# z-prize/2022-entries

Measured on AMD Instinct MI355X. Metric: BLS12-377 G1 MSM point-scalar pairs/s, higher is better.
Workload: dtype u32

## Files before the change

2022-entries_amd/csrc/host_test_api.cpp:

```cpp
#include <stdint.h>
#include <stdio.h>

static long g_check_failures = 0;
static char g_first_failure[256];
static void msm_check_fail(const char* file, int line, const char* cond) {
  if (g_check_failures++ == 0) snprintf(g_first_failure, sizeof g_first_failure, "%s:%d %s", file, line, cond);
}
#define MSM_CHECK(cond) do { if (!(cond)) msm_check_fail(__FILE__, __LINE__, #cond); } while (0)
#define MSM_CHECK_COL_BEGIN() unsigned __int128 chk_col_ = col
#define MSM_CHECK_COL_ADD(x) chk_col_ += (x)
#define MSM_CHECK_COL_END(col) MSM_CHECK(chk_col_ == (unsigned __int128)(col))

#include "host_curve.hpp"
#include "te.hpp"

using namespace msm;

template <class F>
static void t_fe_mul(const uint8_t* a, const uint8_t* b, uint8_t* out) {
  Modulus<F> md;
  Fe x, y, z;
  uint32_t wa[12], wb[12], wo[12];
  memcpy(wa, a, 48);
  memcpy(wb, b, 48);
// ... 655 lines not shown
  uint32_t s[8];
  memcpy(s, scalar, 32);
  const uint32_t levels = fb_levels((uint32_t)w);
  for (uint32_t j = 0; j < levels; j++) out[j] = fb_digit(s, j, (uint32_t)w);
  return (int)levels;
}
int ht_fb_table_level(int curve, const uint8_t* g_img, int w, int level, uint8_t* out, size_t stride) {
  if (!g_img || !out || w < 1 || w > (int)FB_MAX_WINDOW || level < 0 || level >= (int)fb_levels((uint32_t)w) || stride % 4) return -1;
  DISPATCH_C(curve, t_fb_table_level, g_img, w, level, out, stride)
}
int ht_fb_mul(int curve, const uint8_t* g_img, int w, const uint8_t* scalars, size_t n, unsigned flags, uint8_t* out, size_t stride) {
  if (!g_img || (n && (!scalars || !out)) || w < 1 || w > (int)FB_MAX_WINDOW || stride % 4 || (flags & ~3u)) return -1;
  DISPATCH_C(curve, t_fb_mul, g_img, w, scalars, n, flags, out, stride)
}
}
```

2022-entries_amd/csrc/launch.hpp:

```cpp
#pragma once
#include <hip/hip_runtime.h>

#include "host_curve.hpp"
#include "msm_types.hpp"
#include "partition_plan.hpp"
#include "te.hpp"

namespace msm {

template <class E>
struct Launch {
  using El = typename E::T;
  static hipError_t convert_bases(const uint8_t* in, size_t stride, uint32_t n, bool serialized, AffineDevT<El>* out, uint8_t* inf,
                                  hipStream_t st);
  static hipError_t accumulate(const uint2* entries, const uint32_t* n_real, uint32_t K,
                               const AffineDevT<El>* bases, SegOutT<El> out, uint32_t nlanes, hipStream_t st, bool paired = false);
  static hipError_t segreduce(const XyzzDevT<El>* in_slots, const uint32_t* in_keys, uint32_t n_in, uint32_t K, SegOutT<El> out,
                              uint32_t nlanes, uint32_t quad_limit, hipStream_t st, bool paired = false);
  static hipError_t pre_double(const AffineDevT<El>* in, const uint8_t* inf_in, uint32_t n, uint32_t c, XyzzDevT<El>* out, hipStream_t st);
  static hipError_t pre_normalize(const XyzzDevT<El>* in, uint32_t n, uint32_t J, El* prefix, AffineDevT<El>* out, uint8_t* inf_out,
                                  hipStream_t st);
  static hipError_t bucket_reduce(bool first, const XyzzDevT<El>* in_a, const XyzzDevT<El>* in_x, uint32_t n_per_win, uint32_t L,
                                  uint32_t chunks, uint32_t windows, uint32_t out_stride, XyzzDevT<El>* out_a, XyzzDevT<El>* out_x, hipStream_t st,
                                  bool paired = false);
// ... 26 lines not shown
                               const TeAffineDev* bases, SegOut out, uint32_t nlanes, uint32_t* flags, hipStream_t st);
  static hipError_t segreduce(const XyzzDev* in_slots, const uint32_t* in_keys, uint32_t n_in, uint32_t K, SegOut out, uint32_t nlanes,
                              uint32_t quad_limit, uint32_t* flags, hipStream_t st);
  static hipError_t bucket_reduce(bool first, const XyzzDev* in_a, const XyzzDev* in_x, uint32_t n_per_win, uint32_t L, uint32_t chunks,
                                  uint32_t windows, uint32_t out_stride, XyzzDev* out_a, XyzzDev* out_x, uint32_t* flags, hipStream_t st);
  static hipError_t reduce_scan_step(const XyzzDev* in, const XyzzDev* in2, XyzzDev* out, uint32_t nb, uint32_t windows, uint32_t d, uint32_t mode,
                                     uint32_t quad_limit, uint32_t* flags, hipStream_t st);
  static hipError_t sum_bases(const TeAffineDev* bases, const uint8_t* inf, uint32_t first, uint32_t n, uint32_t per_lane, SegOut out, uint32_t nlanes,
                              uint32_t* flags, hipStream_t st);
};

struct PartLaunch {
  static int run(int scalar_field, int scalar_mode, const uint32_t* d_scalars, const uint8_t* d_inf, const PartPlan& p, const PartBuffers& b,
                 hipStream_t st, hipEvent_t mid, hipError_t& err);
  static hipError_t debug_finish(const PartPlan& p, const PartBuffers& b, const uint32_t* slot_keys, uint32_t nslots, hipStream_t st, char* what,
                                 size_t what_len, uint64_t* checks_done);
};

extern template struct Launch<Bls12_377_G1::E>;
extern template struct Launch<Bls12_381_G1::E>;
extern template struct Launch<Bls12_377_G2::E>;
extern template struct Launch<Bls12_381_G2::E>;
extern template struct LaunchPair<Bls12_377_G2::E>;
extern template struct LaunchPair<Bls12_381_G2::E>;

}
```

2022-entries_amd/csrc/msm_engine.hip:

```cpp
#include <hip/hip_runtime.h>

#include <algorithm>
#include <cstdarg>
#include <cstdio>
#include <cstdlib>
#include <cstring>
#include <string.h>
#include <strings.h>

#include <dlfcn.h>

#include <chrono>
#include <condition_variable>
#include <deque>
#include <functional>
#include <memory>
#include <mutex>
#include <stdexcept>
#include <thread>
#include <type_traits>
#include <string>
#include <vector>

#include "../../include/mi355_msm.h"
// ... 225 lines not shown
  return t;
}

struct Plan {
  uint32_t c, windows, half, keybits;
  uint32_t bucket_windows;
  uint32_t levels;
  uint32_t anchor;
  uint64_t entries;
  uint32_t K, nlanes;
  uint32_t segK;
  uint32_t logL0, logL;
  uint32_t T0;
  uint32_t L0;
  uint32_t scan_nb;
  bool reduce_scan;
  bool scan_direct;
};

}

#ifndef MSM_G2_PAIRED_DEFAULT
#define MSM_G2_PAIRED_DEFAULT 31
#endif
constexpr long kDefaultG2Paired = MSM_G2_PAIRED_DEFAULT;

struct RcclState;

struct mi355_msm_ctx {
  int curve = 0;
// ... 23 lines not shown
  long opt_assume_subgroup = 0;
  long opt_anchor = 1;
  bool anchor_armed = false;
  struct AnchorSum {
    size_t n;
    int shift;
    std::vector<uint8_t> pt;
  };
  std::vector<AnchorSum> anchor_sums;
  uint64_t anchor_sums_computed = 0;
  float anchor_sum_ms = 0;
  uint32_t last_anchor = kNoAnchor;
  long opt_reduce_log_chunk = 0, opt_reduce_log_chunk0 = 0;
  long opt_reduce_scan = -1;
  long opt_reduce_fill = 0;
  long opt_twisted_edwards = 1;
  DevBuf te_bases, flags;
  uint32_t* h_flags = nullptr;
  bool te_active = false;
  bool sw_level0_only = false;
  uint64_t te_fallbacks = 0;
  uint32_t te_fallback_streak = 0;
  uint64_t te_demotions = 0;
  uint64_t oom_backoffs = 0;
  uint64_t peer_stagings = 0;
  long opt_force_peer_staging = 0;
  uint32_t last_bucket_windows = 0, last_l1_bits = 0, last_l1_bins = 0, last_passes = 0;
  uint32_t auto_levels = 0;
  uint64_t debug_checks = 0;
  size_t chunk_cap = 0;
  size_t fitted_chunk = 0;
  bool fitted_tables = false;
  uint32_t fitted_c = 0;
  long opt_mem_limit = 0;
  long inject_alloc_failures = 0;
  uint32_t quad_limit = LaunchTe::kDefaultQuadLimit;
  long opt_g2_paired = kDefaultG2Paired;
  std::vector<mi355_msm_ctx*> shards;
  std::vector<size_t> shard_lo;
  long opt_combine = 0;
  RcclState* rccl = nullptr;
  uint64_t rccl_exchanges = 0;
  uint32_t pre_c = 0, pre_windows = 0;
  bool bases_serialized = false;
// ... 60 lines not shown
    if (opt_reduce_log_chunk0) p.logL0 = (uint32_t)opt_reduce_log_chunk0;
    p.logL0 = std::min<uint32_t>(p.logL0, p.c - 1 ? p.c - 1 : 1);
    p.reduce_scan = opt_reduce_scan != 0;
    const uint32_t scan_log = opt_reduce_scan_log ? (uint32_t)opt_reduce_scan_log : 12;
    p.scan_direct = p.reduce_scan && p.half <= (1u << scan_log);
    if (p.reduce_scan && !p.scan_direct) {
      const uint32_t need = ilog2_floor(p.half) - scan_log;
      if (need > 9 || (need > 8 && p.bucket_windows < 8))
        p.reduce_scan = false;
      else if (p.logL0 < need)
        p.logL0 = need;
    }
    p.L0 = 1u << p.logL0;
    p.T0 = ceil_div(p.half, p.L0);
    p.scan_nb = p.T0;
    if (p.reduce_scan && !p.scan_direct && !opt_reduce_log_chunk && !opt_reduce_log_chunk0) {
      const uint64_t kSimds = 1024;
      const uint64_t fill = opt_reduce_fill > 0 ? (uint64_t)opt_reduce_fill : 1;
      const uint64_t waves = ((uint64_t)p.bucket_windows * p.T0 + 63) / 64;
      if (waves < fill * kSimds && p.T0 >= 1024) {
        const uint32_t t_fit = (uint32_t)(fill * kSimds * 64 / p.bucket_windows);
        if (t_fit > p.T0 && t_fit < 2 * fill * p.T0) {
          const uint32_t L = ceil_div(p.half, t_fit);
          if (L >= 8 && L < p.L0) {
            p.L0 = L;
            p.T0 = ceil_div(p.half, L);
            while (p.scan_nb < p.T0) p.scan_nb *= 2;
          }
        }
      }
    }
    return p;
  }
};

namespace {
// ... 248 lines not shown
    const uint64_t sw = (uint64_t)ts.levels * n * 128 * el, inf = (uint64_t)ts.levels * n;
    const uint64_t te_b = te ? (uint64_t)ts.levels * n * sizeof(TeAffineDev) : 0;
    const uint64_t build = te ? 3 * n * 128 + te_b + n * (224 + 56) : sw + n * (224 + 56) * el;
    mi355_msm_ctx tmp;
    tmp.curve = ctx->curve;
    tmp.pre_c = ts.c;
    tmp.pre_windows = ts.levels;
    tmp.opt_window_bits = ctx->opt_window_bits;
    tmp.opt_assume_subgroup = ctx->opt_assume_subgroup;
    tmp.opt_anchor = ctx->opt_anchor;
    tmp.opt_carry = ctx->opt_carry;
    tmp.opt_lane_entries = ctx->opt_lane_entries;
    tmp.opt_seg_entries = ctx->opt_seg_entries;
    tmp.opt_reduce_scan = ctx->opt_reduce_scan;
    tmp.opt_reduce_fill = ctx->opt_reduce_fill;
    const Plan p = tmp.plan(std::min(n, (size_t)1 << 26));
    const uint64_t steady = (te ? n * 128 * el + te_b : sw) + inf + work_bytes(p, el) + n * 32;
    const uint64_t need = std::max(build + inf, steady);
    if (need + (need >> 4) <= avail) return want;
  }
  return -1;
}

bool build_tables_te_streamed(mi355_msm_ctx* ctx, const uint8_t* d_raw, size_t n, size_t stride, int want_levels, hipStream_t st) {
  using C = Bls12_377_G1;
  using E = C::E;
  if (ctx->opt_precompute == 2 && ctx->inject_alloc_failures > 0) {
    ctx->inject_alloc_failures--;
    throw HipFailure((int)hipErrorOutOfMemory, "table allocation failed: out of memory (injected by the inject_alloc_failures test hook)");
  }
// ... 220 lines not shown
  const AffineDev* bases = ctx->bases.as<AffineDev>();
  const uint8_t* inf = ctx->inf.as<uint8_t>();
  uint32_t* flags = ctx->flags.as<uint32_t>();

  HIP_OK(hipEventRecord(ev[0], st));
  PartBuffers gb{};
  gb.entries[0] = ctx->entries[0].as<uint2>();
  gb.entries[1] = ctx->entries[1].as<uint2>();
  gb.matrix = ctx->part_matrix.as<uint32_t>();
  gb.partial = ctx->part_partial.as<uint32_t>();
  gb.segs[0] = ctx->part_segs[0].as<PartSeg>();
  gb.segs[1] = ctx->part_segs[1].as<PartSeg>();
  gb.subjob_first = ctx->part_subjobs.as<uint32_t>();
  gb.counts = ctx->part_counts.as<uint32_t>();
  gb.totals = ctx->part_totals.as<uint32_t>();
  hipError_t gerr = hipSuccess;
  const int scalar_mode = ctx->opt_scalars_montgomery ? SCALARS_FROM_MONT : ctx->opt_scalars_to_montgomery ? SCALARS_TO_MONT : SCALARS_PLAIN;
  const int sorted = PartLaunch::run((ctx->curve == MI355_BLS12_381_G1 || ctx->curve == MI355_BLS12_381_G2) ? 1 : 0, scalar_mode, d_scalars, inf, gp, gb, st,
                                     ev[1], gerr);
  HIP_OK(gerr);
  const uint2* entries = gb.entries[sorted];
  const uint32_t* n_real = gb.totals;
  const bool carry_in = TE && carry && !carry->first;
  if (!carry_in) HIP_OK(hipMemsetAsync(ctx->buckets.p, 0, nbuckets * sizeof(XyzzDev), st));
  HIP_OK(hipEventRecord(ev[2], st));

  SegOut so{ctx->buckets.as<XyzzDev>(), ctx->slots[0].as<XyzzDev>(), ctx->slot_keys[0].as<uint32_t>()};
  so.carry_in = carry_in ? 1u : 0u;
  if constexpr (TE)
    HIP_OK(LaunchTe::accumulate(entries, n_real, p.K, ctx->te_bases.as<TeAffineDev>(), so, p.nlanes, flags, st));
  else
    HIP_OK(Launch<E>::accumulate(entries, n_real, p.K, bases, so, p.nlanes, st, (ctx->opt_g2_paired & 1) != 0));
  HIP_OK(hipEventRecord(ev[3], st));
#ifdef MSM_DEBUG
  {
    char what[320];
    HIP_OK(PartLaunch::debug_finish(gp, gb, ctx->slot_keys[0].as<uint32_t>(), 2 * p.nlanes, st, what, sizeof what, &ctx->debug_checks));
    if (what[0]) throw HipFailure(-2, what);
  }
#endif

  uint32_t n_in = 2 * p.nlanes;
  int cur = 0;
  if (p.nlanes > 1) {
    for (;;) {
      uint32_t nl = ceil_div(n_in, p.segK);
      if (nl > 1 && 2 * (uint64_t)nl >= n_in) bad_arg("fragment merge would not shrink (%u slots, fan-in %u)", n_in, p.segK);
      SegOut o{ctx->buckets.as<XyzzDev>(), ctx->slots[cur ^ 1].as<XyzzDev>(), ctx->slot_keys[cur ^ 1].as<uint32_t>()};
      if constexpr (TE)
        HIP_OK(LaunchTe::segreduce(ctx->slots[cur].as<XyzzDev>(), ctx->slot_keys[cur].as<uint32_t>(), n_in, p.segK, o, nl, ctx->quad_limit, flags, st));
      else
        HIP_OK(Launch<E>::segreduce(ctx->slots[cur].as<XyzzDev>(), ctx->slot_keys[cur].as<uint32_t>(), n_in, p.segK, o, nl, ctx->quad_limit, st,
// ... 37 lines not shown
    HostTail<E>::set_inf(out);
    return true;
  }

  const XyzzDev* sums_src = nullptr;
  uint32_t sums_stride = 1;
  if (p.reduce_scan) {
    uint32_t nb = p.half;
    XyzzDev* bufs[2] = {bucket_src, ctx->red_a[0].as<XyzzDev>()};
    const XyzzDev* a_sums = nullptr;
    if (!p.scan_direct) {
      if (p.scan_nb != p.T0) {
        HIP_OK(hipMemsetAsync(ctx->red_a[0].p, 0, (size_t)p.bucket_windows * p.scan_nb * sizeof(XyzzDev), st));
        HIP_OK(hipMemsetAsync(ctx->red_x[0].p, 0, (size_t)p.bucket_windows * p.scan_nb * sizeof(XyzzDev), st));
      }
      if constexpr (TE)
        HIP_OK(LaunchTe::bucket_reduce(true, nullptr, bucket_src, p.half, p.L0, p.T0, p.bucket_windows, p.scan_nb,
                                       ctx->red_a[0].as<XyzzDev>(), ctx->red_x[0].as<XyzzDev>(), flags, st));
      else
        HIP_OK(Launch<E>::bucket_reduce(true, nullptr, bucket_src, p.half, p.L0, p.T0, p.bucket_windows, p.scan_nb,
                                        ctx->red_a[0].as<XyzzDev>(), ctx->red_x[0].as<XyzzDev>(), st, (ctx->opt_g2_paired & 2) != 0));
      nb = p.scan_nb;
      a_sums = ctx->red_a[0].as<XyzzDev>();
      bufs[0] = ctx->red_x[0].as<XyzzDev>();
      bufs[1] = ctx->red_x[1].as<XyzzDev>();
    }
    int cur = 0;
    auto step = [&](uint32_t d, uint32_t mode) {
      if constexpr (TE)
        HIP_OK(LaunchTe::reduce_scan_step(bufs[cur], a_sums, bufs[cur ^ 1], nb, p.bucket_windows, d, mode, ctx->quad_limit, flags, st));
      else
        HIP_OK(Launch<E>::reduce_scan_step(bufs[cur], a_sums, bufs[cur ^ 1], nb, p.bucket_windows, d, mode, ctx->quad_limit, st, (ctx->opt_g2_paired & 8) != 0));
      cur ^= 1;
    };
    for (uint32_t d = 1; d < nb; d <<= 1) step(d, 0);
    if (a_sums) step(0, 2);
// ... 952 lines not shown
    } else if (k == "reduce_scan_log") {
      if (value != 0 && (value < 6 || value > 18)) bad_arg("reduce_scan_log %ld out of range [6, 18]", value);
      ctx->opt_reduce_scan_log = value;
    } else if (k == "quad_limit") {
      if (value < 0 || value > (1L << 24)) bad_arg("quad_limit %ld out of range [0, 2^24]", value);
      ctx->quad_limit = (uint32_t)value;
    } else if (k == "g2_paired") {
      if (value < 0 || value > 31) bad_arg("g2_paired %ld out of range [0, 31]", value);
      ctx->opt_g2_paired = value;
    } else if (k == "reduce_scan") {
      if (value < -1 || value > 1) bad_arg("reduce_scan %ld out of range [-1, 1]", value);
      ctx->opt_reduce_scan = value;
    } else if (k == "reduce_fill") {
      if (value < 0 || value > 4) bad_arg("reduce_fill %ld out of range [0, 4]", value);
      ctx->opt_reduce_fill = value;
    } else if (k == "reduce_log_chunk0") {
      if (value < 0 || value > 7) bad_arg("reduce_log_chunk0 %ld out of range [1, 7]", value);
      ctx->opt_reduce_log_chunk0 = value;
    } else if (k == "twisted_edwards") {
      ctx->opt_twisted_edwards = value != 0;
    } else if (k == "precompute") {
      if (value < 0 || value > 2) bad_arg("precompute %ld out of range [0, 2]", value);
      ctx->opt_precompute = value;
    } else if (k == "table_levels") {
      if (value < 0 || value > 64) bad_arg("table_levels %ld out of range [0, 64]", value);
      ctx->opt_table_levels = value;
    } else if (k == "scalars_montgomery") {
      if (value != 0 && ctx->opt_scalars_to_montgomery) bad_arg("scalars_montgomery and scalars_to_montgomery exclude each other");
      ctx->opt_scalars_montgomery = value != 0;
    } else if (k == "scalars_to_montgomery") {
// ... 148 lines not shown
      uint32_t v = 0;
      if (ctx->part_totals.p) {
        ensure_device(ctx);
        HIP_OK(hipDeviceSynchronize());
        HIP_OK(hipMemcpy(&v, ctx->part_totals.p, sizeof v, hipMemcpyDeviceToHost));
      }
      *value = v;
    } else if (k == "anchor_sums")
      *value = ctx->anchor_sums_computed;
    else if (k == "anchor_sum_us")
      *value = (uint64_t)(ctx->anchor_sum_ms * 1000.0f);
    else if (k == "oom_backoffs")
      *value = ctx->oom_backoffs;
    else if (k == "debug_checks")
      *value = ctx->debug_checks;
    else if (k == "chunk_cap")
      *value = ctx->chunk_cap;
    else if (k == "device")
      *value = (uint64_t)ctx->device;
    else if (k == "bases")
      *value = ctx->nbases;
    else if (k == "table_levels")
      *value = ctx->pre_c ? ctx->pre_windows : (ctx->nbases ? 1 : 0);
    else if (k == "table_window_bits")
      *value = ctx->pre_c;
    else if (k == "base_bytes")
      *value = ctx->bases.bytes + ctx->te_bases.bytes + ctx->inf.bytes;
    else if (k == "bucket_windows")
      *value = ctx->last_bucket_windows;
    else if (k == "l1_bits")
// ... 196 lines not shown
```

2022-entries_amd/csrc/partition.hip:

```cpp
#include "launch.hpp"
#include "partition.hpp"

namespace msm {

int PartLaunch::run(int scalar_field, int scalar_mode, const uint32_t* d_scalars, const uint8_t* d_inf, const PartPlan& p, const PartBuffers& b,
                    hipStream_t st, hipEvent_t mid, hipError_t& err) {
  if (scalar_field == 1) {
    if (scalar_mode == SCALARS_FROM_MONT) return part_run<Bls12_381_Fr, SCALARS_FROM_MONT>(d_scalars, d_inf, p, b, st, mid, err);
    if (scalar_mode == SCALARS_TO_MONT) return part_run<Bls12_381_Fr, SCALARS_TO_MONT>(d_scalars, d_inf, p, b, st, mid, err);
    return part_run<Bls12_381_Fr, SCALARS_PLAIN>(d_scalars, d_inf, p, b, st, mid, err);
  }
  if (scalar_mode == SCALARS_FROM_MONT) return part_run<Bls12_377_Fr, SCALARS_FROM_MONT>(d_scalars, d_inf, p, b, st, mid, err);
  if (scalar_mode == SCALARS_TO_MONT) return part_run<Bls12_377_Fr, SCALARS_TO_MONT>(d_scalars, d_inf, p, b, st, mid, err);
  return part_run<Bls12_377_Fr, SCALARS_PLAIN>(d_scalars, d_inf, p, b, st, mid, err);
}

hipError_t PartLaunch::debug_finish(const PartPlan& p, const PartBuffers& b, const uint32_t* slot_keys, uint32_t nslots, hipStream_t st, char* what,
                                    size_t what_len, uint64_t* checks_done) {
  if (what && what_len) what[0] = 0;
#ifdef MSM_DEBUG
  uint32_t* const dbg = b.totals + 4;
  const uint32_t key_limit = p.bsets * p.half;
  hipLaunchKernelGGL(k_dbg_check_slots, dim3(part_ceil_div(nslots ? nslots : 1, 256)), dim3(256), 0, st, slot_keys, nslots, key_limit, dbg);
  hipError_t e = hipStreamSynchronize(st);
  if (e != hipSuccess) return e;
  uint32_t h[4 + DBG_WORDS];
  e = hipMemcpy(h, b.totals, sizeof h, hipMemcpyDeviceToHost);
  if (e != hipSuccess) return e;
  const uint32_t* v = h + 4;
  if (checks_done) *checks_done += v[DBG_CHECKS];
  static const char* const names[] = {"", "segment table has a gap or an overlap", "segment table does not end at the entry total",
                                      "an entry carries key bits its level has already resolved", "sorted keys decrease", "a key is out of range",
                                      "a value names a base outside this chunk", "a slot key after the accumulation is neither KEY_NONE nor a valid key"};
  if (v[DBG_DIGITS] != h[0])
    snprintf(what, what_len, "MSM_DEBUG: %u entries were grouped but the scalars hold %u non-zero digits", h[0], v[DBG_DIGITS]);
  else
    for (int i = DBG_SEG_GAP; i <= DBG_SLOT_KEY; i++)
      if (v[i]) {
        snprintf(what, what_len, "MSM_DEBUG: %s (%u violations; n = %u, c = %u, %u windows)", names[i], v[i], p.n, p.c, p.windows);
        break;
      }
#else
  (void)p; (void)b; (void)slot_keys; (void)nslots; (void)st; (void)what_len; (void)checks_done;
#endif
  return hipSuccess;
}

}
```

2022-entries_amd/csrc/partition.hpp:

```cpp
#pragma once
#include <hip/hip_runtime.h>
#include <stdint.h>

#include <algorithm>

#include "digits.hpp"
#include "partition_plan.hpp"

namespace msm {

__device__ __forceinline__ void lds_barrier() {
#ifdef PART_FULL_BARRIER
  __syncthreads();
#else
  asm volatile("s_waitcnt lgkmcnt(0)\n\ts_barrier" ::: "memory");
#endif
}

__device__ __forceinline__ uint32_t wave_incl_scan(uint32_t v) {
#pragma unroll
  for (int d = 1; d < 64; d <<= 1) {
    const uint32_t u = __shfl_up(v, d, 64);
    if ((int)(threadIdx.x & 63) >= d) v += u;
  }
// ... 437 lines not shown
      uint2 e = stage[j];
      const uint32_t hi = e.y >> 16;
      e.y &= 0xffffu;
#ifdef PART_EXP_L1_NOSTORE
      if (e.x == 0x12345678u && e.y == 0x9abcu) out[0] = e;
#elif defined(PART_EXP_L1_OUT4)
      reinterpret_cast<uint32_t*>(out)[offs[hi] + j] = e.x;
#else
      out[offs[hi] + j] = e;
#endif
    }
  }
}


__device__ __forceinline__ bool subjob_range(const PartSeg* __restrict__ segs, const uint32_t* __restrict__ subjob_first, uint32_t nsegs,
                                             uint32_t j, uint32_t& seg, uint32_t& beg, uint32_t& end) {
  if (j >= subjob_first[nsegs]) return false;
  uint32_t lo = 0, hi = nsegs;
  while (hi - lo > 1) {
    const uint32_t mid = (lo + hi) >> 1;
    if (subjob_first[mid] <= j) lo = mid; else hi = mid;
  }
  while (lo + 1 < nsegs && subjob_first[lo + 1] <= j) lo++;
  seg = lo;
  const PartSeg s = segs[seg];
  const uint32_t k = j - subjob_first[seg];
  beg = s.start + k * PART_SUBJOB;
  end = min(s.start + s.len, beg + PART_SUBJOB);
  return beg < end;
// ... 7 lines not shown
  for (uint32_t j = blockIdx.x; j < nsub; j += gridDim.x) {
    uint32_t seg, beg, end;
    const bool live = subjob_range(segs, subjob_first, pp.nsegs, j, seg, beg, end);
    if (!live || part_fused_takes(segs[seg].len)) continue;
    for (uint32_t b = threadIdx.x; b < nb; b += 1024) hist[b] = 0;
    __syncthreads();
    for (uint32_t e = beg + threadIdx.x; e < end; e += 1024) atomicAdd(&hist[(in[e].y >> shift) & (nb - 1)], 1u);
    __syncthreads();
    uint32_t* row = counts + (size_t)j * nb;
    for (uint32_t b = threadIdx.x; b < nb; b += 1024) row[b] = hist[b];
    __syncthreads();
  }
}

__global__ void __launch_bounds__(1024) k_pass_scan(const PartSeg* __restrict__ segs, const uint32_t* __restrict__ subjob_first, PassPlan pp,
                                                    uint32_t* __restrict__ counts, PartSeg* __restrict__ out_segs) {
  __shared__ uint32_t tmp[32];
  const uint32_t s = blockIdx.x, nb = 1u << pp.rb, b = threadIdx.x;
  const PartSeg sg = segs[s];
  if (part_fused_takes(sg.len)) return;
  const uint32_t j0 = subjob_first[s], j1 = subjob_first[s + 1];
  uint32_t tot_b = 0;
  if (b < nb)
    for (uint32_t j = j0; j < j1; j++) tot_b += counts[(size_t)j * nb + b];
  uint32_t tot;
  const uint32_t before = block_excl_scan(tot_b, tmp, tot);
  if (b < nb) {
    uint32_t run = sg.start + before;
    if (out_segs) out_segs[(size_t)s * nb + b] = PartSeg{run, tot_b, sg.key_base + (b << (pp.rem - pp.rb)), 0};
    for (uint32_t j = j0; j < j1; j++) {
      const size_t at = (size_t)j * nb + b;
      const uint32_t v = counts[at];
      counts[at] = run;
      run += v;
    }
  }
}

__global__ void __launch_bounds__(1024) k_pass_subjobs(const PartSeg* __restrict__ segs, uint32_t nsegs, uint32_t* __restrict__ subjob_first,
// ... 101 lines not shown
      if (e.x == 0x12345678u && e.y == 0x9abcu) out[0] = e;
#elif defined(PART_EXP_PS_L2STORE)
      out[(L.dst[bin] + j) & 0x1ffffu] = e;
#elif defined(PART_EXP_PS_OUT4)
      reinterpret_cast<uint32_t*>(out)[L.dst[bin] + j] = e.x;
#else
      out[L.dst[bin] + j] = e;
#endif
    }
  }
}

__global__ void __launch_bounds__(1024, PART_PASS_OCC) k_pass_scatter(const uint2* __restrict__ in, const PartSeg* __restrict__ segs,
                                                          const uint32_t* __restrict__ subjob_first, PassPlan pp, uint32_t gen,
                                                          const uint32_t* __restrict__ positions, uint2* __restrict__ out,
                                                          PartSeg* __restrict__ out_segs) {
  __shared__ PassLds L;
  const uint32_t nb = 1u << pp.rb, shift = pp.rem - pp.rb;
  if (blockIdx.x < gen) {
    const uint32_t nsub = subjob_first[pp.nsegs];
    for (uint32_t j = blockIdx.x; j < nsub; j += gen) {
      uint32_t seg, beg, end;
      const bool live = subjob_range(segs, subjob_first, pp.nsegs, j, seg, beg, end);
      if (!live) continue;
      const PartSeg sg = segs[seg];
      if (part_fused_takes(sg.len)) continue;
      const uint32_t* row = positions + (size_t)j * nb;
      lds_barrier();
      for (uint32_t b = threadIdx.x; b < nb; b += 1024) {
        L.cur[b] = row[b];
        L.cnt[b] = 0;
      }
      lds_barrier();
      pass_scatter_tiles(L, in, out, beg, end, pp, sg.key_base);
    }
    return;
  }
  const uint32_t s = blockIdx.x - gen;
  const PartSeg sg = segs[s];
  if (!part_fused_takes(sg.len)) return;
  if (sg.len == 0) {
    if (out_segs)
      for (uint32_t b = threadIdx.x; b < nb; b += 1024) out_segs[(size_t)s * nb + b] = PartSeg{sg.start, 0, sg.key_base + (b << shift), 0};
    return;
  }
  const uint32_t beg = sg.start, end = sg.start + sg.len;
  for (uint32_t b = threadIdx.x; b < nb; b += 1024) L.cnt[b] = 0;
  lds_barrier();
  {
    uint32_t e = beg + threadIdx.x;
    for (; e + 3 * 1024 < end; e += 4 * 1024) {
      const uint32_t k0 = PART_IN(in, e).y, k1 = PART_IN(in, e + 1024).y, k2 = PART_IN(in, e + 2048).y, k3 = PART_IN(in, e + 3072).y;
      atomicAdd(&L.cnt[(k0 >> shift) & (nb - 1)], 1u);
      atomicAdd(&L.cnt[(k1 >> shift) & (nb - 1)], 1u);
      atomicAdd(&L.cnt[(k2 >> shift) & (nb - 1)], 1u);
      atomicAdd(&L.cnt[(k3 >> shift) & (nb - 1)], 1u);
    }
    for (; e < end; e += 1024) atomicAdd(&L.cnt[(PART_IN(in, e).y >> shift) & (nb - 1)], 1u);
  }
  lds_barrier();
  {
    const uint32_t v = threadIdx.x < nb ? L.cnt[threadIdx.x] : 0;
    uint32_t tot;
    const uint32_t ex = block_excl_scan(v, L.tmp, tot);
    if (threadIdx.x < nb) {
      L.cur[threadIdx.x] = beg + ex;
      L.cnt[threadIdx.x] = 0;
      if (out_segs) out_segs[(size_t)s * nb + threadIdx.x] = PartSeg{beg + ex, v, sg.key_base + (threadIdx.x << shift), 0};
    }
  }
  lds_barrier();
  pass_scatter_tiles(L, in, out, beg, end, pp, sg.key_base);
}

}

namespace msm {

#ifdef MSM_DEBUG
enum { DBG_DIGITS = 0, DBG_SEG_GAP = 1, DBG_SEG_END = 2, DBG_KEY_BITS = 3, DBG_UNSORTED = 4, DBG_KEY_RANGE = 5, DBG_VALUE_RANGE = 6,
       DBG_SLOT_KEY = 7, DBG_CHECKS = 8, DBG_WORDS = 12 };

template <class FR, int MODE, bool FOLD>
__global__ void __launch_bounds__(256) k_dbg_count_digits(const uint32_t* __restrict__ scalars, const uint8_t* __restrict__ inf, PartPlan p,
                                                          uint32_t* __restrict__ dbg) {
  const uint32_t i = blockIdx.x * 256 + threadIdx.x;
  uint32_t count = 0;
  if (i < p.n) {
    ScalarDigits st;
    load_scalar<FR, MODE>(st, scalars, i);
    const bool flip = FOLD ? fold_decision<FR>(st) : false;
    const uint32_t wmask = (1u << p.c) - 1;
    for (uint32_t w = 0; w < p.windows; w++) {
      const uint32_t u = st.s[0] & wmask;
      for (int j = 0; j < 7; j++) st.s[j] = (st.s[j] >> p.c) | (st.s[j + 1] << (32 - p.c));
      st.s[7] >>= p.c;
// ... 29 lines not shown
  for (uint32_t i = blockIdx.x * 256 + threadIdx.x; i < n; i += gridDim.x * 256) {
    const uint2 e = entries[i];
    if (i + 1 < n && entries[i + 1].y < e.y) atomicAdd(&dbg[DBG_UNSORTED], 1u);
    if (e.y >= key_limit) atomicAdd(&dbg[DBG_KEY_RANGE], 1u);
    const uint32_t idx = e.x & 0x7fffffffu;
    if (idx < idx_lo || idx >= idx_hi) atomicAdd(&dbg[DBG_VALUE_RANGE], 1u);
  }
}

__global__ void __launch_bounds__(256) k_dbg_check_slots(const uint32_t* __restrict__ keys, uint32_t n, uint32_t key_limit, uint32_t* __restrict__ dbg) {
  const uint32_t i = blockIdx.x * 256 + threadIdx.x;
  if (i < n && keys[i] != 0xffffffffu && keys[i] >= key_limit) atomicAdd(&dbg[DBG_SLOT_KEY], 1u);
  if (i == 0) atomicAdd(&dbg[DBG_CHECKS], 1u);
}

__global__ void k_dbg_corrupt(uint2* __restrict__ entries, const uint32_t* __restrict__ totals) {
  const uint32_t n = totals[0];
  for (uint32_t i = 0; i + 1 < n; i++)
    if (entries[i].y != entries[i + 1].y) {
      const uint32_t k = entries[i].y;
      entries[i].y = entries[i + 1].y;
      entries[i + 1].y = k;
      return;
    }
}
#endif


#ifndef PART_GEN_GRID
#define PART_GEN_GRID 512u
// ... 57 lines not shown
  PART_MARK("l1_scatter");
  PART_DBG_LEVEL(b.entries[0], b.segs[seg_cur], nsegs, p.lb);
  if (mid) (void)hipEventRecord(mid, st);
  uint32_t rb[4];
  const int np = part_pass_bits(p.lb, rb);
  uint32_t rem = p.lb;
  int cur = 0;
  for (int i = 0; i < np; i++) {
    PassPlan pp{};
    pp.nsegs = (uint32_t)nsegs;
    pp.rem = rem;
    pp.rb = rb[i];
    pp.last = (i == np - 1) ? 1 : 0;
    pp.max_subjobs = part_max_subjobs(entries, nsegs);
    PartSeg* out_segs = pp.last ? nullptr : b.segs[seg_cur ^ 1];
    const bool long_segs = !part_fused_takes((uint32_t)std::min<uint64_t>((uint64_t)p.n * p.levels, 0xffffffffu));
    const uint32_t gen = long_segs ? std::min<uint32_t>(pp.max_subjobs, PART_GEN_GRID) : 0;
    if (long_segs) {
      hipLaunchKernelGGL(k_pass_hist, dim3(std::min<uint32_t>(pp.max_subjobs, 2048u)), dim3(1024), 0, st, b.entries[cur], b.segs[seg_cur], b.subjob_first, pp,
                         b.counts);
      PART_MARK("pass_hist");
      hipLaunchKernelGGL(k_pass_scan, dim3(pp.nsegs), dim3(1024), 0, st, b.segs[seg_cur], b.subjob_first, pp, b.counts, out_segs);
      PART_MARK("pass_scan");
    }
    hipLaunchKernelGGL(k_pass_scatter, dim3(gen + pp.nsegs), dim3(1024), 0, st, b.entries[cur], b.segs[seg_cur], b.subjob_first, pp, gen, b.counts,
                       b.entries[cur ^ 1], out_segs);
    PART_MARK("pass_scatter");
    cur ^= 1;
    rem -= rb[i];
    if (!pp.last) {
      nsegs <<= rb[i];
      seg_cur ^= 1;
      hipLaunchKernelGGL(k_pass_subjobs, dim3(1), dim3(1024), 0, st, b.segs[seg_cur], (uint32_t)nsegs, b.subjob_first, b.totals);
      PART_DBG_LEVEL(b.entries[cur], b.segs[seg_cur], nsegs, rem);
    }
  }
#ifdef MSM_DEBUG
  {
    const uint32_t key_limit = p.bsets * p.half;
    const uint32_t idx_hi = p.idx0 + p.n + (p.levels - 1) * p.table_stride;
    if (getenv("MI355_MSM_DEBUG_CORRUPT")) hipLaunchKernelGGL(k_dbg_corrupt, dim3(1), dim3(1), 0, st, b.entries[cur], b.totals);
    hipLaunchKernelGGL(k_dbg_check_sorted, dim3(2048), dim3(256), 0, st, b.entries[cur], b.totals, key_limit, p.idx0, idx_hi, dbg);
    if (p.fold)
      hipLaunchKernelGGL((k_dbg_count_digits<FR, MODE, true>), dim3(part_ceil_div(p.n, 256)), dim3(256), 0, st, d_scalars, d_inf, p, dbg);
    else
      hipLaunchKernelGGL((k_dbg_count_digits<FR, MODE, false>), dim3(part_ceil_div(p.n, 256)), dim3(256), 0, st, d_scalars, d_inf, p, dbg);
    hipLaunchKernelGGL(k_dbg_check_slots, dim3(1), dim3(256), 0, st, b.totals, 0u, 0u, dbg);
  }
#endif
  err = hipGetLastError();
  return cur;
}

}
```

2022-entries_amd/csrc/partition_plan.hpp:

```cpp
#pragma once
#include <hip/hip_runtime.h>
#include <stddef.h>
#include <stdint.h>

#include <algorithm>

namespace msm {

enum ScalarMode : int {
  SCALARS_PLAIN = 0,
  SCALARS_FROM_MONT = 1,
  SCALARS_TO_MONT = 2,
};

constexpr int PART_TILE = 8192;
constexpr int PART_THREADS = 1024;
constexpr int PART_PER_THREAD = PART_TILE / PART_THREADS;
#ifndef PART_MAX_HB_V
#define PART_MAX_HB_V 10
#endif
constexpr int PART_MAX_HB = PART_MAX_HB_V;
constexpr int PART_MAX_RB = 10;
constexpr uint32_t PART_SUBJOB = 192u << 10;
#ifndef PART_PTILE_V
// ... 118 lines not shown
  s.segs_a = s.segs_b = (size_t)max_segs * sizeof(PartSeg);
  s.subjob_first = (size_t)(max_sj + 1) * 4;
  s.counts = (size_t)max_counts * 4;
  s.totals = 64;
  return s;
}

struct PartBuffers {
  uint2* entries[2];
  uint32_t* matrix;
  uint32_t* partial;
  PartSeg* segs[2];
  uint32_t* subjob_first;
  uint32_t* counts;
  uint32_t* totals;
};


}
```

Before: 657.8 million.

## Zero empty buckets during scatter and shrink top-window bucket reduction

Drops the full hipMemsetAsync over the bucket array. Instead, the final partition pass zeroes only the buckets that receive no sorted entries, inside the scan and scatter kernels. Separately, the first bucket-reduce level now treats the top window apart from the others, reducing only the buckets its limited scalar bits can reach, and the chunk-fit heuristic excludes that window. This cuts memory traffic and wasted point additions, at the cost of more complex indexing, scattered writes inside the partition kernels, and a debug checker to catch stale buckets.

```diff
diff --git a/2022-entries_amd/csrc/host_test_api.cpp b/2022-entries_amd/csrc/host_test_api.cpp
--- a/2022-entries_amd/csrc/host_test_api.cpp
+++ b/2022-entries_amd/csrc/host_test_api.cpp
@@ -693,3 +693,9 @@
   DISPATCH_C(curve, t_fb_mul, g_img, w, scalars, n, flags, out, stride)
 }
 }
+
+#include "top_window.hpp"
+extern "C" int ht_top_window_buckets(int c, int windows, int levels, long anchor) {
+  if (c < 2 || c > 24 || windows < 1 || levels < 0) return -1;
+  return (int)msm::part_top_window_buckets((uint32_t)c, (uint32_t)windows, (uint32_t)levels, anchor < 0 ? 0xffffffffu : (uint32_t)anchor);
+}
diff --git a/2022-entries_amd/csrc/launch.hpp b/2022-entries_amd/csrc/launch.hpp
--- a/2022-entries_amd/csrc/launch.hpp
+++ b/2022-entries_amd/csrc/launch.hpp
@@ -64,7 +64,7 @@
   static int run(int scalar_field, int scalar_mode, const uint32_t* d_scalars, const uint8_t* d_inf, const PartPlan& p, const PartBuffers& b,
                  hipStream_t st, hipEvent_t mid, hipError_t& err);
   static hipError_t debug_finish(const PartPlan& p, const PartBuffers& b, const uint32_t* slot_keys, uint32_t nslots, hipStream_t st, char* what,
-                                 size_t what_len, uint64_t* checks_done);
+                                 size_t what_len, uint64_t* checks_done, uint64_t* empty_checks_done = nullptr);
 };
 
 extern template struct Launch<Bls12_377_G1::E>;
diff --git a/2022-entries_amd/csrc/msm_engine.hip b/2022-entries_amd/csrc/msm_engine.hip
--- a/2022-entries_amd/csrc/msm_engine.hip
+++ b/2022-entries_amd/csrc/msm_engine.hip
@@ -263,6 +263,7 @@
   uint32_t T0;
   uint32_t L0;
   uint32_t scan_nb;
+  uint32_t top_buckets;
   bool reduce_scan;
   bool scan_direct;
 };
@@ -316,6 +317,7 @@
   long opt_reduce_log_chunk = 0, opt_reduce_log_chunk0 = 0;
   long opt_reduce_scan = -1;
   long opt_reduce_fill = 0;
+  long opt_reduce_top = 1;
   long opt_twisted_edwards = 1;
   DevBuf te_bases, flags;
   uint32_t* h_flags = nullptr;
@@ -330,6 +332,7 @@
   uint32_t last_bucket_windows = 0, last_l1_bits = 0, last_l1_bins = 0, last_passes = 0;
   uint32_t auto_levels = 0;
   uint64_t debug_checks = 0;
+  uint64_t debug_empty_checks = 0;
   size_t chunk_cap = 0;
   size_t fitted_chunk = 0;
   bool fitted_tables = false;
@@ -420,12 +423,16 @@
     p.L0 = 1u << p.logL0;
     p.T0 = ceil_div(p.half, p.L0);
     p.scan_nb = p.T0;
+    p.top_buckets = p.half;
+    if (opt_reduce_top && p.levels == 1 && p.reduce_scan && !p.scan_direct)
+      p.top_buckets = part_top_window_buckets(p.c, p.windows, p.levels, opt_assume_subgroup ? PART_NO_ANCHOR : p.anchor);
+    const uint32_t full_windows = p.top_buckets < p.half ? p.bucket_windows - 1 : p.bucket_windows;
     if (p.reduce_scan && !p.scan_direct && !opt_reduce_log_chunk && !opt_reduce_log_chunk0) {
       const uint64_t kSimds = 1024;
       const uint64_t fill = opt_reduce_fill > 0 ? (uint64_t)opt_reduce_fill : 1;
-      const uint64_t waves = ((uint64_t)p.bucket_windows * p.T0 + 63) / 64;
-      if (waves < fill * kSimds && p.T0 >= 1024) {
-        const uint32_t t_fit = (uint32_t)(fill * kSimds * 64 / p.bucket_windows);
+      const uint64_t waves = ((uint64_t)full_windows * p.T0 + 63) / 64;
+      if (full_windows && waves < fill * kSimds && p.T0 >= 1024) {
+        const uint32_t t_fit = (uint32_t)(fill * kSimds * 64 / full_windows);
         if (t_fit > p.T0 && t_fit < 2 * fill * p.T0) {
           const uint32_t L = ceil_div(p.half, t_fit);
           if (L >= 8 && L < p.L0) {
@@ -704,6 +711,7 @@
     tmp.opt_seg_entries = ctx->opt_seg_entries;
     tmp.opt_reduce_scan = ctx->opt_reduce_scan;
     tmp.opt_reduce_fill = ctx->opt_reduce_fill;
+    tmp.opt_reduce_top = ctx->opt_reduce_top;
     const Plan p = tmp.plan(std::min(n, (size_t)1 << 26));
     const uint64_t steady = (te ? n * 128 * el + te_b : sw) + inf + work_bytes(p, el) + n * 32;
     const uint64_t need = std::max(build + inf, steady);
@@ -954,6 +962,12 @@
   gb.subjob_first = ctx->part_subjobs.as<uint32_t>();
   gb.counts = ctx->part_counts.as<uint32_t>();
   gb.totals = ctx->part_totals.as<uint32_t>();
+  const bool carry_in = TE && carry && !carry->first;
+  if (!carry_in) {
+    static_assert(sizeof(XyzzDev) % 16 == 0 && sizeof(XyzzDev) / 16 <= 64, "the grouping zeroes a bucket record with one lane per 16 bytes");
+    gb.zero_buckets = ctx->buckets.as<uint4>();
+    gb.zero_rec16 = (uint32_t)(sizeof(XyzzDev) / 16);
+  }
   hipError_t gerr = hipSuccess;
   const int scalar_mode = ctx->opt_scalars_montgomery ? SCALARS_FROM_MONT : ctx->opt_scalars_to_montgomery ? SCALARS_TO_MONT : SCALARS_PLAIN;
   const int sorted = PartLaunch::run((ctx->curve == MI355_BLS12_381_G1 || ctx->curve == MI355_BLS12_381_G2) ? 1 : 0, scalar_mode, d_scalars, inf, gp, gb, st,
@@ -961,8 +975,6 @@
   HIP_OK(gerr);
   const uint2* entries = gb.entries[sorted];
   const uint32_t* n_real = gb.totals;
-  const bool carry_in = TE && carry && !carry->first;
-  if (!carry_in) HIP_OK(hipMemsetAsync(ctx->buckets.p, 0, nbuckets * sizeof(XyzzDev), st));
   HIP_OK(hipEventRecord(ev[2], st));
 
   SegOut so{ctx->buckets.as<XyzzDev>(), ctx->slots[0].as<XyzzDev>(), ctx->slot_keys[0].as<uint32_t>()};
@@ -975,7 +987,7 @@
 #ifdef MSM_DEBUG
   {
     char what[320];
-    HIP_OK(PartLaunch::debug_finish(gp, gb, ctx->slot_keys[0].as<uint32_t>(), 2 * p.nlanes, st, what, sizeof what, &ctx->debug_checks));
+    HIP_OK(PartLaunch::debug_finish(gp, gb, ctx->slot_keys[0].as<uint32_t>(), 2 * p.nlanes, st, what, sizeof what, &ctx->debug_checks, &ctx->debug_empty_checks));
     if (what[0]) throw HipFailure(-2, what);
   }
 #endif
@@ -1043,12 +1055,29 @@
         HIP_OK(hipMemsetAsync(ctx->red_a[0].p, 0, (size_t)p.bucket_windows * p.scan_nb * sizeof(XyzzDev), st));
         HIP_OK(hipMemsetAsync(ctx->red_x[0].p, 0, (size_t)p.bucket_windows * p.scan_nb * sizeof(XyzzDev), st));
       }
-      if constexpr (TE)
-        HIP_OK(LaunchTe::bucket_reduce(true, nullptr, bucket_src, p.half, p.L0, p.T0, p.bucket_windows, p.scan_nb,
-                                       ctx->red_a[0].as<XyzzDev>(), ctx->red_x[0].as<XyzzDev>(), flags, st));
-      else
-        HIP_OK(Launch<E>::bucket_reduce(true, nullptr, bucket_src, p.half, p.L0, p.T0, p.bucket_windows, p.scan_nb,
-                                        ctx->red_a[0].as<XyzzDev>(), ctx->red_x[0].as<XyzzDev>(), st, (ctx->opt_g2_paired & 2) != 0));
+      auto first_level = [&](uint32_t w0, uint32_t wins, uint32_t n_per_win, uint32_t L, uint32_t chunks) {
+        XyzzDev* const out_a = ctx->red_a[0].as<XyzzDev>() + (size_t)w0 * p.scan_nb;
+        XyzzDev* const out_x = ctx->red_x[0].as<XyzzDev>() + (size_t)w0 * p.scan_nb;
+        if constexpr (TE)
+          HIP_OK(LaunchTe::bucket_reduce(true, nullptr, bucket_src + (size_t)w0 * p.half, n_per_win, L, chunks, wins, p.scan_nb, out_a, out_x, flags, st));
+        else
+          HIP_OK(Launch<E>::bucket_reduce(true, nullptr, bucket_src + (size_t)w0 * p.half, n_per_win, L, chunks, wins, p.scan_nb, out_a, out_x, st,
+                                          (ctx->opt_g2_paired & 2) != 0));
+      };
+      if (p.top_buckets < p.half) {
+        const uint32_t top = p.bucket_windows - 1;
+        if (top) first_level(0, top, p.half, p.L0, p.T0);
+        if (p.scan_nb == p.T0) {
+          HIP_OK(hipMemsetAsync(ctx->red_a[0].as<XyzzDev>() + (size_t)top * p.scan_nb, 0, (size_t)p.scan_nb * sizeof(XyzzDev), st));
+          HIP_OK(hipMemsetAsync(ctx->red_x[0].as<XyzzDev>() + (size_t)top * p.scan_nb, 0, (size_t)p.scan_nb * sizeof(XyzzDev), st));
+        }
+        if (p.top_buckets) {
+          const uint32_t L = p.top_buckets >= 64 * p.L0 ? p.L0 : ceil_div(p.top_buckets, 64);
+          first_level(top, 1, p.top_buckets, L, ceil_div(p.top_buckets, L));
+        }
+      } else {
+        first_level(0, p.bucket_windows, p.half, p.L0, p.T0);
+      }
       nb = p.scan_nb;
       a_sums = ctx->red_a[0].as<XyzzDev>();
       bufs[0] = ctx->red_x[0].as<XyzzDev>();
@@ -2031,6 +2060,9 @@
     } else if (k == "reduce_fill") {
       if (value < 0 || value > 4) bad_arg("reduce_fill %ld out of range [0, 4]", value);
       ctx->opt_reduce_fill = value;
+    } else if (k == "reduce_top") {
+      if (value < 0 || value > 1) bad_arg("reduce_top %ld out of range [0, 1]", value);
+      ctx->opt_reduce_top = value;
     } else if (k == "reduce_log_chunk0") {
       if (value < 0 || value > 7) bad_arg("reduce_log_chunk0 %ld out of range [1, 7]", value);
       ctx->opt_reduce_log_chunk0 = value;
@@ -2209,6 +2241,8 @@
       *value = ctx->oom_backoffs;
     else if (k == "debug_checks")
       *value = ctx->debug_checks;
+    else if (k == "debug_empty_checks")
+      *value = ctx->debug_empty_checks;
     else if (k == "chunk_cap")
       *value = ctx->chunk_cap;
     else if (k == "device")
diff --git a/2022-entries_amd/csrc/partition.hip b/2022-entries_amd/csrc/partition.hip
--- a/2022-entries_amd/csrc/partition.hip
+++ b/2022-entries_amd/csrc/partition.hip
@@ -16,7 +16,7 @@
 }
 
 hipError_t PartLaunch::debug_finish(const PartPlan& p, const PartBuffers& b, const uint32_t* slot_keys, uint32_t nslots, hipStream_t st, char* what,
-                                    size_t what_len, uint64_t* checks_done) {
+                                    size_t what_len, uint64_t* checks_done, uint64_t* empty_checks_done) {
   if (what && what_len) what[0] = 0;
 #ifdef MSM_DEBUG
   uint32_t* const dbg = b.totals + 4;
@@ -40,8 +40,12 @@
         snprintf(what, what_len, "MSM_DEBUG: %s (%u violations; n = %u, c = %u, %u windows)", names[i], v[i], p.n, p.c, p.windows);
         break;
       }
+  if (what && !what[0] && v[DBG_STALE_BUCKET])
+    snprintf(what, what_len, "MSM_DEBUG: a bucket without a sorted entry is not all-zero before the accumulation (%u violations; n = %u, c = %u, %u windows)",
+             v[DBG_STALE_BUCKET], p.n, p.c, p.windows);
+  if (empty_checks_done) *empty_checks_done += v[DBG_EMPTY_CHECKS];
 #else
-  (void)p; (void)b; (void)slot_keys; (void)nslots; (void)st; (void)what_len; (void)checks_done;
+  (void)p; (void)b; (void)slot_keys; (void)nslots; (void)st; (void)what_len; (void)checks_done; (void)empty_checks_done;
 #endif
   return hipSuccess;
 }
diff --git a/2022-entries_amd/csrc/partition.hpp b/2022-entries_amd/csrc/partition.hpp
--- a/2022-entries_amd/csrc/partition.hpp
+++ b/2022-entries_amd/csrc/partition.hpp
@@ -475,6 +475,22 @@
 }
 
 
+__device__ __forceinline__ void zero_records(uint4* __restrict__ zb, uint32_t rec16, uint32_t first, uint32_t count, uint32_t tid, uint32_t nthreads) {
+  uint4* const at = zb + (size_t)first * rec16;
+  const uint32_t n16 = count * rec16;
+  for (uint32_t i = tid; i < n16; i += nthreads) at[i] = make_uint4(0, 0, 0, 0);
+}
+__device__ __forceinline__ void wave_zero_empty(uint4* __restrict__ zb, uint32_t rec16, uint32_t bucket, bool empty) {
+  uint64_t m = __builtin_amdgcn_ballot_w64(empty);
+  const uint32_t lane = threadIdx.x & 63;
+  while (m) {
+    const int l = __ffsll((unsigned long long)m) - 1;
+    m &= m - 1;
+    const uint32_t b = __shfl(bucket, l, 64);
+    if (lane < rec16) zb[(size_t)b * rec16 + lane] = make_uint4(0, 0, 0, 0);
+  }
+}
+
 __device__ __forceinline__ bool subjob_range(const PartSeg* __restrict__ segs, const uint32_t* __restrict__ subjob_first, uint32_t nsegs,
                                              uint32_t j, uint32_t& seg, uint32_t& beg, uint32_t& end) {
   if (j >= subjob_first[nsegs]) return false;
@@ -512,7 +528,8 @@
 }
 
 __global__ void __launch_bounds__(1024) k_pass_scan(const PartSeg* __restrict__ segs, const uint32_t* __restrict__ subjob_first, PassPlan pp,
-                                                    uint32_t* __restrict__ counts, PartSeg* __restrict__ out_segs) {
+                                                    uint32_t* __restrict__ counts, PartSeg* __restrict__ out_segs, uint4* __restrict__ zb,
+                                                    uint32_t rec16) {
   __shared__ uint32_t tmp[32];
   const uint32_t s = blockIdx.x, nb = 1u << pp.rb, b = threadIdx.x;
   const PartSeg sg = segs[s];
@@ -521,6 +538,7 @@
   uint32_t tot_b = 0;
   if (b < nb)
     for (uint32_t j = j0; j < j1; j++) tot_b += counts[(size_t)j * nb + b];
+  if (zb) wave_zero_empty(zb, rec16, sg.key_base + b, b < nb && tot_b == 0);
   uint32_t tot;
   const uint32_t before = block_excl_scan(tot_b, tmp, tot);
   if (b < nb) {
@@ -652,7 +670,7 @@
 __global__ void __launch_bounds__(1024, PART_PASS_OCC) k_pass_scatter(const uint2* __restrict__ in, const PartSeg* __restrict__ segs,
                                                           const uint32_t* __restrict__ subjob_first, PassPlan pp, uint32_t gen,
                                                           const uint32_t* __restrict__ positions, uint2* __restrict__ out,
-                                                          PartSeg* __restrict__ out_segs) {
+                                                          PartSeg* __restrict__ out_segs, uint4* __restrict__ zb, uint32_t rec16) {
   __shared__ PassLds L;
   const uint32_t nb = 1u << pp.rb, shift = pp.rem - pp.rb;
   if (blockIdx.x < gen) {
@@ -680,6 +698,7 @@
   if (sg.len == 0) {
     if (out_segs)
       for (uint32_t b = threadIdx.x; b < nb; b += 1024) out_segs[(size_t)s * nb + b] = PartSeg{sg.start, 0, sg.key_base + (b << shift), 0};
+    if (zb) zero_records(zb, rec16, sg.key_base, nb, threadIdx.x, 1024);
     return;
   }
   const uint32_t beg = sg.start, end = sg.start + sg.len;
@@ -701,6 +720,7 @@
     const uint32_t v = threadIdx.x < nb ? L.cnt[threadIdx.x] : 0;
     uint32_t tot;
     const uint32_t ex = block_excl_scan(v, L.tmp, tot);
+    if (zb) wave_zero_empty(zb, rec16, sg.key_base + threadIdx.x, threadIdx.x < nb && v == 0);
     if (threadIdx.x < nb) {
       L.cur[threadIdx.x] = beg + ex;
       L.cnt[threadIdx.x] = 0;
@@ -717,7 +737,7 @@
 
 #ifdef MSM_DEBUG
 enum { DBG_DIGITS = 0, DBG_SEG_GAP = 1, DBG_SEG_END = 2, DBG_KEY_BITS = 3, DBG_UNSORTED = 4, DBG_KEY_RANGE = 5, DBG_VALUE_RANGE = 6,
-       DBG_SLOT_KEY = 7, DBG_CHECKS = 8, DBG_WORDS = 12 };
+       DBG_SLOT_KEY = 7, DBG_CHECKS = 8, DBG_STALE_BUCKET = 9, DBG_EMPTY_CHECKS = 10, DBG_WORDS = 12 };
 
 template <class FR, int MODE, bool FOLD>
 __global__ void __launch_bounds__(256) k_dbg_count_digits(const uint32_t* __restrict__ scalars, const uint8_t* __restrict__ inf, PartPlan p,
@@ -777,6 +797,29 @@
   if (i == 0) atomicAdd(&dbg[DBG_CHECKS], 1u);
 }
 
+__global__ void __launch_bounds__(256) k_dbg_check_empty(const uint2* __restrict__ entries, const uint32_t* __restrict__ totals, uint32_t key_limit,
+                                                         const uint4* __restrict__ zb, uint32_t rec16, uint32_t* __restrict__ dbg) {
+  const uint32_t n = totals[0];
+  for (uint32_t k = blockIdx.x * 256 + threadIdx.x; k < key_limit; k += gridDim.x * 256) {
+    uint32_t lo = 0, hi = n;
+    while (lo < hi) {
+      const uint32_t mid = lo + ((hi - lo) >> 1);
+      if (entries[mid].y < k) lo = mid + 1; else hi = mid;
+    }
+    if (lo < n && entries[lo].y == k) continue;
+    uint32_t nz = 0;
+    for (uint32_t i = 0; i < rec16; i++) {
+      const uint4 q = zb[(size_t)k * rec16 + i];
+      nz |= q.x | q.y | q.z | q.w;
+    }
+    if (nz) atomicAdd(&dbg[DBG_STALE_BUCKET], 1u);
+  }
+  if (blockIdx.x == 0 && threadIdx.x == 0) {
+    atomicAdd(&dbg[DBG_CHECKS], 1u);
+    atomicAdd(&dbg[DBG_EMPTY_CHECKS], 1u);
+  }
+}
+
 __global__ void k_dbg_corrupt(uint2* __restrict__ entries, const uint32_t* __restrict__ totals) {
   const uint32_t n = totals[0];
   for (uint32_t i = 0; i + 1 < n; i++)
@@ -864,17 +907,18 @@
     pp.last = (i == np - 1) ? 1 : 0;
     pp.max_subjobs = part_max_subjobs(entries, nsegs);
     PartSeg* out_segs = pp.last ? nullptr : b.segs[seg_cur ^ 1];
+    uint4* const zb = pp.last ? b.zero_buckets : nullptr;
     const bool long_segs = !part_fused_takes((uint32_t)std::min<uint64_t>((uint64_t)p.n * p.levels, 0xffffffffu));
     const uint32_t gen = long_segs ? std::min<uint32_t>(pp.max_subjobs, PART_GEN_GRID) : 0;
     if (long_segs) {
       hipLaunchKernelGGL(k_pass_hist, dim3(std::min<uint32_t>(pp.max_subjobs, 2048u)), dim3(1024), 0, st, b.entries[cur], b.segs[seg_cur], b.subjob_first, pp,
                          b.counts);
       PART_MARK("pass_hist");
-      hipLaunchKernelGGL(k_pass_scan, dim3(pp.nsegs), dim3(1024), 0, st, b.segs[seg_cur], b.subjob_first, pp, b.counts, out_segs);
+      hipLaunchKernelGGL(k_pass_scan, dim3(pp.nsegs), dim3(1024), 0, st, b.segs[seg_cur], b.subjob_first, pp, b.counts, out_segs, zb, b.zero_rec16);
       PART_MARK("pass_scan");
     }
     hipLaunchKernelGGL(k_pass_scatter, dim3(gen + pp.nsegs), dim3(1024), 0, st, b.entries[cur], b.segs[seg_cur], b.subjob_first, pp, gen, b.counts,
-                       b.entries[cur ^ 1], out_segs);
+                       b.entries[cur ^ 1], out_segs, zb, b.zero_rec16);
     PART_MARK("pass_scatter");
     cur ^= 1;
     rem -= rb[i];
@@ -891,6 +935,8 @@
     const uint32_t idx_hi = p.idx0 + p.n + (p.levels - 1) * p.table_stride;
     if (getenv("MI355_MSM_DEBUG_CORRUPT")) hipLaunchKernelGGL(k_dbg_corrupt, dim3(1), dim3(1), 0, st, b.entries[cur], b.totals);
     hipLaunchKernelGGL(k_dbg_check_sorted, dim3(2048), dim3(256), 0, st, b.entries[cur], b.totals, key_limit, p.idx0, idx_hi, dbg);
+    if (b.zero_buckets)
+      hipLaunchKernelGGL(k_dbg_check_empty, dim3(2048), dim3(256), 0, st, b.entries[cur], b.totals, key_limit, b.zero_buckets, b.zero_rec16, dbg);
     if (p.fold)
       hipLaunchKernelGGL((k_dbg_count_digits<FR, MODE, true>), dim3(part_ceil_div(p.n, 256)), dim3(256), 0, st, d_scalars, d_inf, p, dbg);
     else
diff --git a/2022-entries_amd/csrc/partition_plan.hpp b/2022-entries_amd/csrc/partition_plan.hpp
--- a/2022-entries_amd/csrc/partition_plan.hpp
+++ b/2022-entries_amd/csrc/partition_plan.hpp
@@ -4,6 +4,8 @@
 #include <stdint.h>
 
 #include <algorithm>
+
+#include "top_window.hpp"
 
 namespace msm {
 
@@ -156,6 +158,8 @@
   uint32_t* subjob_first;
   uint32_t* counts;
   uint32_t* totals;
+  uint4* zero_buckets;
+  uint32_t zero_rec16;
 };
 
 
diff --git a/2022-entries_amd/csrc/top_window.hpp b/2022-entries_amd/csrc/top_window.hpp
--- /dev/null
+++ b/2022-entries_amd/csrc/top_window.hpp
@@ -0,0 +1,18 @@
+#pragma once
+#include <stdint.h>
+
+#include <algorithm>
+
+namespace msm {
+
+inline uint32_t part_top_window_buckets(uint32_t c, uint32_t windows, uint32_t levels, uint32_t anchor) {
+  const uint32_t half = 1u << (c - 1);
+  if (levels > 1 || windows < 2) return half;
+  const uint32_t below = (windows - 1) * c;
+  const uint32_t top_bits = below < 256 ? 256 - below : 0;
+  if (top_bits >= c) return half;
+  const uint64_t most = ((1ull << top_bits) - 1) + (anchor == windows - 2 ? 0 : 1);
+  return (uint32_t)std::min<uint64_t>(most, half);
+}
+
+}
```

Measured after the change: 661.6 million, median of 6. Within noise of the previous version (+0.6%).
